# hanseongbugi/ORB_SLAM3_Study_kr

Measured on AMD Instinct MI355X. Metric: local-BA windows/sec (50 KF, 10k pts, 10 LM iters) + ORB matches/sec; 1/2/4/8 GPU, higher is better.
Workload: dtype f64; 1 GPU; BASELINE.json configs[1]: synthetic stereo local BA, 50 optimisable + 10 fixed KF, 10k landmarks (~75k stereo edges), optimize(10) with the reference's stop rules; windows_per_gpu=512, global_windows=512, streams_per_gpu=2, parallelism=independent windows, w mod 1

## Files before the change

### orb_slam3_study_kr_amd/csrc/lba_device.hip

```cpp
#include "common.h"
#include <type_traits>
#include <cstdlib>
#include <cstdio>
#include <atomic>
#include <chrono>
#include <thread>
#include "lba_math.h"
#include "ldlt_block.h"
#include "big_solve.h"
#include "schur_plan.h"
#include "lba_pack.h"
#include "lba_pack_device.h"
#include "g2o_lm.h"
#include <algorithm>
#include <cfloat>
#include <cmath>
#include <cstring>
#include <vector>

namespace osh {

constexpr int kResidualSplit = 1;
constexpr int kSolveThreadsBatch = 256, kSolveThreadsLatency = 512;
constexpr int kPoseRec = 21;
// ... 299 lines not shown
      const int e = pbase + tid;
      double hl[9];
#pragma unroll
      for (int k = 0; k < 9; ++k) hl[k] = 0.0;
      if (e < e1) {
        double qt[7], cam[5], R[9], X[3], Xc[3], Q[6], g[3], rho0;
        fetch_pose(staged, sh_pose, poses, cams, le.ip[p], qt, cam, R);
#pragma unroll
        for (int k = 0; k < 3; ++k) X[k] = sh_X[(le.il[p] - ch.lm0) * 3 + k];
        const double rec[4] = {le.ra[p].x, le.ra[p].y, le.rb[p].x, le.rb[p].y};
        win_edge_core<KB8>(wd, bv, (size_t)wd.edge_off + e, rec, qt, cam, R, X, Xc, Q, g, rho0);
        chi_acc += rho0;
        dev::core_landmark_side<KB8>(Q, g, R, hl);
      }
#pragma unroll
      for (int k = 0; k < 9; ++k) sh_c[k * kChunkEdges + tid] = hl[k];
      __syncthreads();
      if (tid < nl) {
        const int lo = max(my_lo, pbase), hi = min(my_hi, pbase + kChunkEdges);
        for (int x = lo; x < hi; ++x) {
#pragma unroll
          for (int k = 0; k < 9; ++k) acc[k] += sh_c[k * kChunkEdges + x - pbase];
        }
      }
      __syncthreads();
    }
  }
  double dmax = 0.0;
  if (tid < nl) {
    const size_t gl = (size_t)wd.pt_off + ch.lm0 + tid;
#pragma unroll
    for (int k = 0; k < 6; ++k) bv.Hll[gl * 6 + k] = acc[k];
#pragma unroll
    for (int k = 0; k < 3; ++k) bv.bl[gl * 3 + k] = acc[6 + k];
    dmax = fmax(fabs(acc[0]), fmax(fabs(acc[3]), fabs(acc[5])));
    if (lambda_known) {
      double dl[9];
      dev::landmark_factor(acc, acc + 6, st.lambda, dl);
#pragma unroll
      for (int k = 0; k < 9; ++k) bv.DL[gl * 9 + k] = dl[k];
    }
  }
  const double chi = block_sum(chi_acc, sh4);
  dmax = block_max(dmax, sh4);
  if (tid == 0) { bv.chi_lin[blockIdx.x] = chi; bv.dmax_lin[blockIdx.x] = dmax; }
}

typedef double f64x4 __attribute__((ext_vector_type(4)));
constexpr int kSiLm = 8;
constexpr int kSiRows = 6 * kItemPoses;
constexpr int kSiImage = 32 * 49;

template <bool SYM, bool KB8>
__global__ __launch_bounds__(64, KB8 ? 1 : 2) void k_schur_fused(BatchView bv, int item_base, int mode) {
  __shared__ double shA[(SYM && !KB8) ? kSiImage : kSiRows * (3 * kSiLm + 1)];
  __shared__ double shB[SYM ? 1 : kSiRows * (3 * kSiLm + 1)];
  __shared__ double shPose[(SYM ? 1 : 2) * 8 * kPoseRec];
  __shared__ int shP[64 + 8];
  const int item_idx = item_base + blockIdx.x;
  const SItem it = bv.sitems[item_idx];
  const WinDesc wd = bv.win[it.win];
  const LmView st = lm_view(bv.lm, it.win);
  if (!st.active) return;
  const bool do_hpp = SYM && (mode == 0 ? st.need_lin != 0 : (st.lin_now != 0 && st.iter > 0));
  const bool do_schur = mode != 0;
  if (!do_hpp && !do_schur) return;
  const int lane = threadIdx.x;
  const int nx = it.shape & 0xff, ny = (it.shape >> 8) & 0xff;
  const int TX = (6 * nx + 15) >> 4, TY = (6 * ny + 15) >> 4;
  shP[lane] = bv.spair[(size_t)item_idx * 64 + lane];
  if (lane < 8) shP[64 + lane] = bv.scslot[(size_t)item_idx * 8 + lane];
  {
    const double* poses = bv.pose_state[st.sel] + (size_t)wd.pose_off * 7;
    const double* cams = bv.pose_cam + (size_t)wd.pose_off * 5;
    const int side = lane >> 3, s8 = lane & 7;
    if (side < (SYM ? 1 : 2)) {
      const int ip = side == 0 ? bv.sposex[(size_t)item_idx * 8 + s8] : bv.sposey[(size_t)item_idx * 8 + s8];
      double qt[7], cam[5], Rm[9];
#pragma unroll
      for (int k = 0; k < 7; ++k) qt[k] = ip >= 0 ? poses[(size_t)ip * 7 + k] : 0.0;
#pragma unroll
      for (int k = 0; k < 5; ++k) cam[k] = ip >= 0 ? cams[(size_t)ip * 5 + k] : 0.0;
      dev::quat_to_R(qt, Rm);
      double* dst = shPose + (side * 8 + s8) * kPoseRec;
#pragma unroll
      for (int k = 0; k < 7; ++k) dst[k] = qt[k];
#pragma unroll
      for (int k = 0; k < 5; ++k) dst[7 + k] = cam[k];
#pragma unroll
      for (int k = 0; k < 9; ++k) dst[12 + k] = Rm[k];
    }
  }
  const SRec* __restrict__ recs = bv.srecs + it.rec_off;
  const double* pts = bv.pt_state[st.sel] + (size_t)wd.pt_off * 3;
  const double* DL = bv.DL + (size_t)wd.pt_off * 9;
  const int mrow = lane & 15, mk = lane >> 4;
  using std::integral_constant;

  auto body = [&](auto lmc, auto psc) __attribute__((always_inline)) {
    constexpr int LM = decltype(lmc)::value, PS = decltype(psc)::value;
    constexpr int KS = 3 * LM + 1;
    constexpr int KST = (3 * LM) / 4;
    static_assert(LM * PS <= 64 && (3 * LM) % 4 == 0 && ((6 * PS + 15) / 16) * 16 * KS <= ((SYM && !KB8) ? kSiImage : kSiRows * (3 * kSiLm + 1)), "chunk mapping");
    const int l = lane / PS, s = lane - l * PS;
    const bool lane_on = LM * PS == 64 || l < LM;
    f64x4 acc[3][3];
#pragma unroll
    for (int a = 0; a < 3; ++a)
#pragma unroll
      for (int b = 0; b < 3; ++b) acc[a][b] = (f64x4){0.0, 0.0, 0.0, 0.0};
    double csum[6] = {0, 0, 0, 0, 0, 0};
    double H[21], hb[6];
#pragma unroll
    for (int k = 0; k < 21; ++k) H[k] = 0.0;
#pragma unroll
    for (int k = 0; k < 6; ++k) hb[k] = 0.0;
    if (PS < 8) {
      for (int idx = lane; idx < (((6 * PS + 15) / 16) * 16 - 6 * PS) * KS; idx += 64) shA[6 * PS * KS + idx] = 0.0;
    }

    struct Dat { double2 ex[2]; double2 ey[2]; double X[3]; double dl[9]; };
    const int last_rec = it.n_lm - 1;
    const size_t last_edge = (size_t)wd.edge_off + (size_t)max(wd.E - 1, 0);
    auto load_rec = [&](int c0, int4& ra, int4& rb) {
      const int4* src = reinterpret_cast<const int4*>(recs + min(c0 + l, last_rec));
      ra = src[0]; rb = src[1];
    };
    auto slot_of = [&](unsigned lo, unsigned hi) { return (((s < 4) ? lo : hi) >> (8 * (s & 3))) & 0xffu; };
    auto edge_of = [&](const int4& ra, unsigned o) { return min((size_t)wd.edge_off + (size_t)(ra.y + (o != kAbsent ? (int)o : 0)), last_edge); };
    auto load_dat = [&](const int4& ra, const int4& rb, Dat& d) {
      const double2* src = reinterpret_cast<const double2*>(bv.e_rec + edge_of(ra, slot_of((unsigned)ra.z, (unsigned)ra.w)) * 4);
      d.ex[0] = src[0]; d.ex[1] = src[1];
      if (!SYM) {
        const double2* sy = reinterpret_cast<const double2*>(bv.e_rec + edge_of(ra, slot_of((unsigned)rb.x, (unsigned)rb.y)) * 4);
        d.ey[0] = sy[0]; d.ey[1] = sy[1];
      }
#pragma unroll
      for (int k = 0; k < 3; ++k) d.X[k] = pts[(size_t)ra.x * 3 + k];
      if (do_schur) {
#pragma unroll
        for (int k = 0; k < 9; ++k) d.dl[k] = DL[(size_t)ra.x * 9 + k];
      }
    };
    auto side_rows = [&](int side, bool present, const int4& ra, unsigned o, const double2* er, const Dat& d, double* img) __attribute__((always_inline)) {
      const double* ps = shPose + (side * 8 + s) * kPoseRec;
      double qt[7], cam[5], Rm[9];
#pragma unroll
      for (int k = 0; k < 7; ++k) qt[k] = ps[k];
#pragma unroll
      for (int k = 0; k < 5; ++k) cam[k] = ps[7 + k];
#pragma unroll
      for (int k = 0; k < 9; ++k) Rm[k] = ps[12 + k];
      const double rec[4] = {er[0].x, er[0].y, er[1].x, er[1].y};
      double Xc[3], Q[6], g[3], rho0;
      win_edge_core<KB8>(wd, bv, edge_of(ra, o), rec, qt, cam, Rm, d.X, Xc, Q, g, rho0);
#pragma unroll
      for (int k = 0; k < 6; ++k) Q[k] = present ? Q[k] : 0.0;
#pragma unroll
      for (int k = 0; k < 3; ++k) g[k] = present ? g[k] : 0.0;
      if (SYM && do_hpp && side == 0) dev::core_pose_side<KB8>(Xc, Q, g, H, hb);
      if (do_schur) {
        double WF[18];
        dev::core_WF<KB8>(Xc, Q, Rm, d.dl, WF);
        double* row = img + (6 * s) * KS + 3 * l;
        if (lane_on) {
#pragma unroll
          for (int r = 0; r < 6; ++r) { row[r * KS + 0] = WF[r * 3]; row[r * KS + 1] = WF[r * 3 + 1]; row[r * KS + 2] = WF[r * 3 + 2]; }
        }
        if (SYM) {
#pragma unroll
          for (int r = 0; r < 6; ++r) csum[r] += WF[r * 3] * d.dl[6] + WF[r * 3 + 1] * d.dl[7] + WF[r * 3 + 2] * d.dl[8];
        }
      }
    };
    auto park = [&](int c0, const int4& ra, const int4& rb, const Dat& d) __attribute__((always_inline)) {
      const bool valid = lane_on && (c0 + l) < it.n_lm;
      const unsigned xo = valid ? slot_of((unsigned)ra.z, (unsigned)ra.w) : kAbsent;
      wave_sync();
      side_rows(0, xo != kAbsent, ra, xo, d.ex, d, shA);
      if (!SYM) {
        const unsigned yo = valid ? slot_of((unsigned)rb.x, (unsigned)rb.y) : kAbsent;
        side_rows(1, yo != kAbsent, ra, yo, d.ey, d, shB);
      }
    };
    auto multiply_t = [&](auto txc, auto tyc) {
      constexpr int TXc = decltype(txc)::value, TYc = decltype(tyc)::value;
      const double* imgB = SYM ? shA : shB;
#pragma unroll
      for (int ks = 0; ks < KST; ++ks) {
        double a[3], b[3];
#pragma unroll
        for (int t = 0; t < 3; ++t) {
          a[t] = (t < TXc) ? shA[(16 * t + mrow) * KS + 4 * ks + mk] : 0.0;
          b[t] = SYM ? a[t] : ((t < TYc) ? imgB[(16 * t + mrow) * KS + 4 * ks + mk] : 0.0);
        }
#pragma unroll
        for (int ti = 0; ti < 3; ++ti)
#pragma unroll
          for (int tj = SYM ? ti : 0; tj < 3; ++tj)
            if (ti < TXc && tj < TYc) acc[ti][tj] = __builtin_amdgcn_mfma_f64_16x16x4f64(a[ti], b[tj], acc[ti][tj], 0, 0, 0);
        if (ks & 1) __builtin_amdgcn_sched_barrier(0);
      }
    };
    auto multiply_cross = [&]() {
#pragma unroll
      for (int ks = 0; ks < KST; ++ks) {
        double a[3], b[3];
#pragma unroll
        for (int t = 0; t < 3; ++t) {
          a[t] = (t < TX) ? shA[(16 * t + mrow) * KS + 4 * ks + mk] : 0.0;
          b[t] = (t < TY) ? shB[(16 * t + mrow) * KS + 4 * ks + mk] : 0.0;
        }
#pragma unroll
        for (int ti = 0; ti < 3; ++ti)
#pragma unroll
          for (int tj = 0; tj < 3; ++tj)
            if (ti < TX && tj < TY) acc[ti][tj] = __builtin_amdgcn_mfma_f64_16x16x4f64(a[ti], b[tj], acc[ti][tj], 0, 0, 0);
      }
    };
    int4 rc0, rc1, rn0, rn1;
    Dat d;
    load_rec(0, rc0, rc1);
    load_rec(LM, rn0, rn1);
    load_dat(rc0, rc1, d);
    wave_sync();
    auto chunk_loop = [&](auto txc) {
      for (int c0 = 0; c0 < it.n_lm; c0 += LM) {
        park(c0, rc0, rc1, d);
        wave_sync();
        rc0 = rn0; rc1 = rn1;
        load_dat(rc0, rc1, d);
        load_rec(c0 + 2 * LM, rn0, rn1);
        if (do_schur) {
          if (SYM) multiply_t(txc, txc); else multiply_cross();
        }
      }
    };
    if (SYM && do_schur) {
      if (PS > 5 && TX == 3) chunk_loop(integral_constant<int, 3>{});
      else if (PS > 2 && TX == 2) chunk_loop(integral_constant<int, 2>{});
      else chunk_loop(integral_constant<int, 1>{});
    } else {
      chunk_loop(integral_constant<int, 0>{});
    }
    wave_sync();
    if (do_schur) {
#pragma unroll
      for (int ti = 0; ti < 3; ++ti)
#pragma unroll
        for (int tj = SYM ? ti : 0; tj < 3; ++tj) {
          if (ti < TX && tj < TY) {
            const int C = 16 * tj + (lane & 15);
            const int sb = C / 6, cc = C - 6 * sb;
#pragma unroll
            for (int reg = 0; reg < 4; ++reg) {
              const int R = 16 * ti + (lane >> 4) + 4 * reg;
              const int sa = R / 6, rr = R - 6 * sa;
              const int slot = shP[sa * 8 + sb];
              if (slot >= 0) bv.contrib[(size_t)slot * 36 + rr * 6 + cc] = acc[ti][tj][reg];
            }
          }
        }
      if (SYM) {
        if (lane_on) {
#pragma unroll
          for (int r = 0; r < 6; ++r) shA[l * (6 * PS) + 6 * s + r] = csum[r];
        }
        wave_sync();
        if (lane < 6 * PS) {
          double v = 0.0;
#pragma unroll
          for (int k = 0; k < LM; ++k) v += shA[k * (6 * PS) + lane];
          const int sa = lane / 6;
          const int slot = shP[64 + sa];
          if (slot >= 0) bv.ccontrib[(size_t)slot * 6 + (lane - 6 * sa)] = v;
        }
        wave_sync();
      }
    }
    if (SYM && do_hpp) {
#pragma unroll
      for (int half = 0; half < 2; ++half) {
        const int k0 = half * 14, nk = half ? 13 : 14;
        wave_sync();
#pragma unroll
        for (int k = 0; k < 14; ++k) {
          const int kk = k0 + k;
          if (k < nk) shA[k * 64 + lane] = (kk < 21) ? H[kk < 21 ? kk : 0] : hb[(kk - 21) < 0 ? 0 : ((kk - 21) > 5 ? 5 : (kk - 21))];
        }
        wave_sync();
        for (int o = lane; o < PS * nk; o += 64) {
          const int k = o / PS, sa = o - k * PS;
          const int slot = shP[64 + sa];
          if (slot >= 0) {
            double v = 0.0;
#pragma unroll
            for (int ll = 0; ll < LM; ++ll) v += shA[k * 64 + ll * PS + sa];
            bv.hcontrib[(size_t)slot * 27 + k0 + k] = v;
          }
        }
      }
    }
  };
  if constexpr (SYM && !KB8) {
    if (nx <= 4) body(integral_constant<int, 16>{}, integral_constant<int, 4>{});
    else if (nx == 5) body(integral_constant<int, 12>{}, integral_constant<int, 5>{});
    else body(integral_constant<int, kSiLm>{}, integral_constant<int, 8>{});
  } else {
    body(integral_constant<int, kSiLm>{}, integral_constant<int, 8>{});
  }
}

template <bool DEEP>
__global__ __launch_bounds__(256) void k_schur_reduce(BatchView bv) {
  const int t = threadIdx.x / 36, el = threadIdx.x - 36 * t;
  const int idx = blockIdx.x * 7 + t;
  if (t >= 7 || idx >= bv.n_rblk) return;
  const RBlk rb = bv.rblk[idx];
  const WinDesc wd = bv.win[rb.win];
  const LmView st = lm_view(bv.lm, rb.win);
  if (!st.active) return;
  const int i = rb.ij & 0xffff, j = (rb.ij >> 16) & 0xffff;
  if (j == 0xffff) {
    if (el >= 6) return;
    const size_t gp = (size_t)wd.fpose_off + i;
    double v = bv.bp[gp * 6 + el];
    const double* c = bv.ccontrib + (size_t)rb.start * 6 + el;
    int k = 0;
    if constexpr (DEEP) {
      for (; k + 24 <= rb.count; k += 24) {
        double t[24];
#pragma unroll
        for (int u = 0; u < 24; ++u) t[u] = c[(size_t)(k + u) * 6];
        __builtin_amdgcn_sched_barrier(0);
#pragma unroll
        for (int u = 0; u < 24; ++u) v -= t[u];
      }
    }
    for (; k + 8 <= rb.count; k += 8) {
      double t[8];
#pragma unroll
      for (int u = 0; u < 8; ++u) t[u] = c[(size_t)(k + u) * 6];
      __builtin_amdgcn_sched_barrier(0);
#pragma unroll
      for (int u = 0; u < 8; ++u) v -= t[u];
    }
    for (; k < rb.count; ++k) v -= c[(size_t)k * 6];
    bv.bs[gp * 6 + el] = v;
    return;
  }
  if (bv.pose_lo && i < bv.pose_lo[wd.fpose_off + j]) return;
  const int r = el / 6, cc = el - 6 * r;
  double v = 0.0;
  if (i == j) v = bv.Hpp[((size_t)wd.fpose_off + i) * 36 + el] + ((r == cc) ? st.lambda : 0.0);
  const double* c = bv.contrib + (size_t)rb.start * 36 + el;
  int k = 0;
  if constexpr (DEEP) {
    for (; k + 24 <= rb.count; k += 24) {
      double t[24];
#pragma unroll
      for (int u = 0; u < 24; ++u) t[u] = c[(size_t)(k + u) * 36];
      __builtin_amdgcn_sched_barrier(0);
#pragma unroll
      for (int u = 0; u < 24; ++u) v -= t[u];
    }
  }
  for (; k + 8 <= rb.count; k += 8) {
    double t[8];
#pragma unroll
    for (int u = 0; u < 8; ++u) t[u] = c[(size_t)(k + u) * 36];
    __builtin_amdgcn_sched_barrier(0);
#pragma unroll
    for (int u = 0; u < 8; ++u) v -= t[u];
  }
  for (; k < rb.count; ++k) v -= c[(size_t)k * 36];
  bv.S[wd.S_off + (size_t)(6 * i + r) * wd.n + 6 * j + cc] = v;
}

__global__ __launch_bounds__(64) void k_pose_reduce(BatchView bv, int mode) {
  const int gp = blockIdx.x * 2 + (threadIdx.x >> 5);
  const int k = threadIdx.x & 31;
  if (gp >= bv.n_fposes) return;
  const int w = bv.fpose_win[gp];
  const LmView st = lm_view(bv.lm, w);
  if (!st.active || !(mode == 0 ? st.need_lin != 0 : (st.lin_now != 0 && st.iter > 0))) return;
  const I2 rg = bv.pose_crange[gp];
  double a = 0.0;
  if (k < 27) {
    const double* src = bv.hcontrib + (size_t)rg.x * 27 + k;
    int c = 0;
    for (; c + 16 <= rg.y; c += 16) {
      double t[16];
#pragma unroll
      for (int u = 0; u < 16; ++u) t[u] = src[(size_t)(c + u) * 27];
      __builtin_amdgcn_sched_barrier(0);
#pragma unroll
      for (int u = 0; u < 16; ++u) a += t[u];
    }
    for (; c + 4 <= rg.y; c += 4) {
      const double v0 = src[(size_t)c * 27], v1 = src[(size_t)(c + 1) * 27], v2 = src[(size_t)(c + 2) * 27], v3 = src[(size_t)(c + 3) * 27];
      a += v0; a += v1; a += v2; a += v3;
    }
    for (; c < rg.y; ++c) a += src[(size_t)c * 27];
    if (k < 21) {
      int r = 0, rem = k;
      while (rem >= 6 - r) { rem -= 6 - r; ++r; }
      const int cc = r + rem;
      double* Ho = bv.Hpp + (size_t)gp * 36;
      Ho[r * 6 + cc] = a;
      Ho[cc * 6 + r] = a;
    } else {
      bv.bp[(size_t)gp * 6 + (k - 21)] = a;
    }
  }
  __shared__ double shd[64];
  shd[threadIdx.x] = fabs(a);
  wave_sync();
  if (k == 0) {
    const double* d = shd + (threadIdx.x & 32);
    bv.dmax_pose[gp] = fmax(fmax(fmax(d[0], d[6]), fmax(d[11], d[15])), fmax(d[18], d[20]));
  }
}

template <int NT>
__device__ void solve_tail(BatchView& bv, const WinDesc& wd, LmState& st, const double* xs, double* shw, bool ok) {
  const int tid = threadIdx.x, n = wd.n;
  double* xp = bv.xp + (size_t)wd.fpose_off * 6;
  for (int k = tid; k < n; k += NT) xp[k] = xs[k];
  __syncthreads();
  const int cur = st.sel, tr_sel = st.sel ^ 1;
  const double lambda = st.lambda;
  double sc = 0.0;
  for (int i = tid; i < wd.P; i += NT) {
    double u[6], qin[7], qout[7];
#pragma unroll
    for (int k = 0; k < 6; ++k) u[k] = xs[6 * i + k];
#pragma unroll
    for (int k = 0; k < 7; ++k) qin[k] = bv.pose_state[cur][((size_t)wd.pose_off + i) * 7 + k];
    dev::pose_oplus(u, qin, qout);
#pragma unroll
    for (int k = 0; k < 7; ++k) bv.pose_state[tr_sel][((size_t)wd.pose_off + i) * 7 + k] = qout[k];
    const double* bpi = bv.bp + ((size_t)wd.fpose_off + i) * 6;
#pragma unroll
    for (int k = 0; k < 6; ++k) sc += u[k] * (lambda * u[k] + bpi[k]);
  }
  sc = dev::wave_sum(sc);
  if ((tid & 63) == 0) shw[tid >> 6] = sc;
  __syncthreads();
  if (tid == 0) {
    double tot = 0.0;
    for (int k = 0; k < NT / 64; ++k) tot += shw[k];
    st.scale_pose = tot; st.solve_ok = ok ? 1 : 0;
  }
}

template <int NB, int NT>
__global__ __launch_bounds__(NT) void k_solve(BatchView bv, int W) {
  constexpr int kSolveThreads = NT;
  extern __shared__ __attribute__((aligned(16))) double sh[];
  const int w = blockIdx.x;
  const WinDesc& wd = bv.win[w];
  LmState& st = bv.lm[w];
  if (!st.active) return;
  const int n = wd.n;
  double* A = bv.S + wd.S_off;
  double* rhs = bv.bs + (size_t)wd.fpose_off * 6;
  double *xs, *shw;
  const bool ok = ldlt_solve_block<NB, kSolveThreads>(A, rhs, n, W, sh, xs, shw, bv.pose_lo ? bv.pose_lo + wd.fpose_off : nullptr);
  solve_tail<kSolveThreads>(bv, wd, st, xs, shw, ok);
}

__global__ __launch_bounds__(256) void k_big_finish(BatchView bv, int w, const int* fail) {
  __shared__ double shw[8];
  const WinDesc& wd = bv.win[w];
  LmState& st = bv.lm[w];
  if (!st.active) return;
  double* x = bv.bs + (size_t)wd.fpose_off * 6;
  const bool ok = *fail == 0;
  if (!ok) {
    for (int k = threadIdx.x; k < wd.n; k += 256) x[k] = 0.0;
    __syncthreads();
  }
  solve_tail<256>(bv, wd, st, x, shw, ok);
}

template <bool KB8, bool F32>
__global__ __launch_bounds__(kBlock) void k_backsub(BatchView bv) {
  extern __shared__ __attribute__((aligned(16))) double sh_bs[];
  double* sh_c = sh_bs;
  double* sh4 = sh_bs + 3 * kChunkEdges;
  double* sh_X = sh4 + 4;
  double* sh_x = sh_X + 3 * kBlock;
  const Chunk ch = bv.chunks[blockIdx.x];
  const WinDesc wd = bv.win[ch.win];
  const LmView st = lm_view(bv.lm, ch.win);
  if (!st.active) return;
  const int tid = threadIdx.x;
  const int n = wd.n;
  const double* poses = bv.pose_state[st.sel] + (size_t)wd.pose_off * 7;
  const double* cams = bv.pose_cam + (size_t)wd.pose_off * 5;
  const double* pts = bv.pt_state[st.sel] + (size_t)wd.pt_off * 3;
  const bool staged = wd.P <= kLdsPoses;
  const double* xp = bv.xp + (size_t)wd.fpose_off * 6;
  double* sh_pose = sh_x + (staged ? n : 0);
  const int* lmo = bv.lm_off + wd.lmoff_off;
  const int e0 = lmo[ch.lm0], e1 = lmo[ch.lm1];
  const int nl = ch.lm1 - ch.lm0;
  const double lambda = st.lambda;
  double acc[3] = {0, 0, 0};
  int my_lo = 0, my_hi = 0;
  double F[6], b3[3], Xcur[3];
#pragma unroll
  for (int k = 0; k < 6; ++k) F[k] = 0.0;
  b3[0] = b3[1] = b3[2] = 0.0; Xcur[0] = Xcur[1] = Xcur[2] = 0.0;
  if (tid < nl) {
    const size_t gl = (size_t)wd.pt_off + ch.lm0 + tid;
    my_lo = lmo[ch.lm0 + tid]; my_hi = lmo[ch.lm0 + tid + 1];
#pragma unroll
    for (int k = 0; k < 6; ++k) F[k] = bv.DL[gl * 9 + k];
#pragma unroll
    for (int k = 0; k < 3; ++k) { b3[k] = bv.bl[gl * 3 + k]; Xcur[k] = pts[(size_t)(ch.lm0 + tid) * 3 + k]; }
  }
  for (int base = e0; base < e1; base += kChunkMaxEdges) {
    LaneEdges le;
    load_lane_edges<F32>(bv, wd, base, e1, tid, le);
    if (base == e0) {
      stage_points(sh_X, pts, ch.lm0, nl, tid);
      if (staged) {
        for (int k = tid; k < n; k += kBlock) sh_x[k] = xp[k];
        stage_poses(sh_pose, poses, cams, wd.P, tid, kBlock);
      }
      __syncthreads();
    }
#pragma unroll
    for (int p = 0; p < kPasses; ++p) {
      const int pbase = base + p * kChunkEdges;
      if (pbase >= e1) break;
      const int e = pbase + tid;
      double c[3] = {0, 0, 0};
      if (e < e1 && le.ip[p] < wd.P) {
        const int ip = le.ip[p];
        double qt[7], R[9], cam[5], X[3], Xc[3], Q[6], g[3], rho0, x6[6];
        fetch_pose(staged, sh_pose, poses, cams, ip, qt, cam, R);
#pragma unroll
        for (int k = 0; k < 6; ++k) x6[k] = staged ? sh_x[6 * ip + k] : xp[6 * ip + k];
#pragma unroll
        for (int k = 0; k < 3; ++k) X[k] = sh_X[(le.il[p] - ch.lm0) * 3 + k];
        const double rec[4] = {le.ra[p].x, le.ra[p].y, le.rb[p].x, le.rb[p].y};
        win_edge_core<KB8>(wd, bv, (size_t)wd.edge_off + e, rec, qt, cam, R, X, Xc, Q, g, rho0);
        dev::core_backsub<KB8>(Xc, Q, R, x6, c);
      }
      sh_c[tid] = c[0]; sh_c[kChunkEdges + tid] = c[1]; sh_c[2 * kChunkEdges + tid] = c[2];
      __syncthreads();
      if (tid < nl) {
        const int lo = max(my_lo, pbase), hi = min(my_hi, pbase + kChunkEdges);
        for (int x = lo; x < hi; ++x) {
          acc[0] += sh_c[x - pbase]; acc[1] += sh_c[kChunkEdges + x - pbase]; acc[2] += sh_c[2 * kChunkEdges + x - pbase];
        }
      }
      __syncthreads();
    }
  }
  double sc = 0.0;
  if (tid < nl) {
    const size_t gl = (size_t)wd.pt_off + ch.lm0 + tid;
    const double b0 = b3[0], b1 = b3[1], b2 = b3[2];
    const double c0 = b0 + acc[0], c1 = b1 + acc[1], c2 = b2 + acc[2];
    double xl[3];
    if (st.solve_ok) {
      const double t0 = F[0] * c0, t1 = F[1] * c0 + F[3] * c1, t2 = F[2] * c0 + F[4] * c1 + F[5] * c2;
      xl[0] = F[0] * t0 + F[1] * t1 + F[2] * t2;
      xl[1] = F[3] * t1 + F[4] * t2;
      xl[2] = F[5] * t2;
    } else {
      xl[0] = xl[1] = xl[2] = 0.0;
    }
    double* Xt = bv.pt_state[st.sel ^ 1] + gl * 3;
    Xt[0] = Xcur[0] + xl[0]; Xt[1] = Xcur[1] + xl[1]; Xt[2] = Xcur[2] + xl[2];
    sc = xl[0] * (lambda * xl[0] + b0) + xl[1] * (lambda * xl[1] + b1) + xl[2] * (lambda * xl[2] + b2);
  }
  sc = block_sum(sc, sh4);
  if (tid == 0) bv.scale_part[blockIdx.x] = sc;
  __syncthreads();
  if (tid < nl) {
    const double* Xt = bv.pt_state[st.sel ^ 1] + ((size_t)wd.pt_off + ch.lm0 + tid) * 3;
    sh_X[tid * 3] = Xt[0]; sh_X[tid * 3 + 1] = Xt[1]; sh_X[tid * 3 + 2] = Xt[2];
  }
  const double* poses_t = bv.pose_state[st.sel ^ 1] + (size_t)wd.pose_off * 7;
  const bool staged_t = (wd.P + wd.F) <= kLdsPoses;
  double* sh_pose_t = sh_pose + (staged ? wd.P * kPoseRec : 0);
  if (staged_t) stage_poses(sh_pose_t, poses_t, cams, wd.P + wd.F, tid, kBlock);
  __syncthreads();
  double chi_acc = 0.0;
  for (int base = e0; base < e1; base += kChunkMaxEdges) {
    LaneEdges le;
    load_lane_edges<F32>(bv, wd, base, e1, tid, le);
#pragma unroll
    for (int p = 0; p < kPasses; ++p) {
      const int e = base + p * kChunkEdges + tid;
      if (e < e1) {
        double qt[7], cam[5], R[9], X[3];
        fetch_pose(staged_t, sh_pose_t, poses_t, cams, le.ip[p], qt, cam, R);
#pragma unroll
        for (int k = 0; k < 3; ++k) X[k] = sh_X[(le.il[p] - ch.lm0) * 3 + k];
        const double rec[4] = {le.ra[p].x, le.ra[p].y, le.rb[p].x, le.rb[p].y};
        double cl, cr;
// ... 857 lines not shown
```

Before: 13070 windows/s.

## Add specialized cross-pair Schur kernel path for narrow column tiles with MFMA pipelining

Adds a dedicated code path for non-symmetric Schur off-diagonal blocks when the row tile has more than five poses and the column tile has at most four. It builds WF images for row and column poses in shared memory, software-pipelines record and data loads ahead of the compute passes, and accumulates with f64 MFMA tiles sized to the narrow column count. The aim is to avoid wasted MFMA work and padding that the generic 8x8 body spends on small column tiles. In exchange it adds a large specialised code path with more register pressure and extra indexing complexity.

```diff
diff --git a/orb_slam3_study_kr_amd/csrc/lba_device.hip b/orb_slam3_study_kr_amd/csrc/lba_device.hip
--- a/orb_slam3_study_kr_amd/csrc/lba_device.hip
+++ b/orb_slam3_study_kr_amd/csrc/lba_device.hip
@@ -625,6 +625,135 @@
       }
     }
   };
+  auto cross_pairs = [&](auto tyc) __attribute__((always_inline)) {
+    constexpr int TYc = decltype(tyc)::value;
+    constexpr int KS = 3 * kSiLm + 1, KSB = 3 * 16 + 1, KST = (3 * kSiLm) / 4;
+    static_assert(16 * TYc <= 32 && kSiRows * KS <= sizeof(shA) / sizeof(double) && 24 * KSB <= sizeof(shB) / sizeof(double), "image sizes");
+    const int l = lane >> 3, s = lane & 7;
+    const int lc = lane >> 2, sc = lane & 3;
+    f64x4 acc[3][TYc];
+#pragma unroll
+    for (int a = 0; a < 3; ++a)
+#pragma unroll
+      for (int b = 0; b < TYc; ++b) acc[a][b] = (f64x4){0.0, 0.0, 0.0, 0.0};
+
+    struct SDat { double2 e[2]; double X[3]; double dl[9]; };
+    const int last_rec = it.n_lm - 1;
+    const size_t last_edge = (size_t)wd.edge_off + (size_t)max(wd.E - 1, 0);
+    auto edge_of = [&](const int4& ra, unsigned o) { return min((size_t)wd.edge_off + (size_t)(ra.y + (o != kAbsent ? (int)o : 0)), last_edge); };
+    auto row_slot = [&](const int4& ra) { return (unsigned)((((unsigned long long)(unsigned)ra.w << 32) | (unsigned)ra.z) >> (8 * s)) & 0xffu; };
+    auto col_slot = [&](const int4& rb) { return ((unsigned)rb.x >> (8 * sc)) & 0xffu; };
+    auto load_row_rec = [&](int c0, int4& ra) { ra = *reinterpret_cast<const int4*>(recs + min(c0 + l, last_rec)); };
+    auto load_col_rec = [&](int p0, int4& ra, int4& rb) {
+      const int4* src = reinterpret_cast<const int4*>(recs + min(p0 + lc, last_rec));
+      ra = src[0]; rb = src[1];
+    };
+    auto load_dat = [&](const int4& ra, unsigned o, SDat& d) {
+      const double2* src = reinterpret_cast<const double2*>(bv.e_rec + edge_of(ra, o) * 4);
+      d.e[0] = src[0]; d.e[1] = src[1];
+#pragma unroll
+      for (int k = 0; k < 3; ++k) d.X[k] = pts[(size_t)ra.x * 3 + k];
+#pragma unroll
+      for (int k = 0; k < 9; ++k) d.dl[k] = DL[(size_t)ra.x * 9 + k];
+    };
+    auto wf_rows = [&](const double* ps, bool present, size_t ge, const SDat& d, double* row, int ks) __attribute__((always_inline)) {
+      double qt[7], cam[5], Rm[9];
+#pragma unroll
+      for (int k = 0; k < 7; ++k) qt[k] = ps[k];
+#pragma unroll
+      for (int k = 0; k < 5; ++k) cam[k] = ps[7 + k];
+#pragma unroll
+      for (int k = 0; k < 9; ++k) Rm[k] = ps[12 + k];
+      const double rec[4] = {d.e[0].x, d.e[0].y, d.e[1].x, d.e[1].y};
+      double Xc[3], Q[6], g[3], rho0;
+      win_edge_core<KB8>(wd, bv, ge, rec, qt, cam, Rm, d.X, Xc, Q, g, rho0);
+#pragma unroll
+      for (int k = 0; k < 6; ++k) Q[k] = present ? Q[k] : 0.0;
+      double WF[18];
+      dev::core_WF<KB8>(Xc, Q, Rm, d.dl, WF);
+#pragma unroll
+      for (int r = 0; r < 6; ++r) { row[r * ks + 0] = WF[r * 3]; row[r * ks + 1] = WF[r * 3 + 1]; row[r * ks + 2] = WF[r * 3 + 2]; }
+    };
+    auto row_pass = [&](int c0, const int4& ra, const SDat& d) __attribute__((always_inline)) {
+      const unsigned o = (c0 + l) < it.n_lm ? row_slot(ra) : kAbsent;
+      wf_rows(shPose + s * kPoseRec, o != kAbsent, edge_of(ra, o), d, shA + (6 * s) * KS + 3 * l, KS);
+    };
+    auto col_pass = [&](int p0, const int4& ra, const int4& rb, const SDat& d) __attribute__((always_inline)) {
+      const unsigned o = (p0 + lc) < it.n_lm ? col_slot(rb) : kAbsent;
+      wf_rows(shPose + (8 + sc) * kPoseRec, o != kAbsent, edge_of(ra, o), d, shB + (6 * sc) * KSB + 3 * lc, KSB);
+    };
+    auto multiply = [&](int cb) __attribute__((always_inline)) {
+#pragma unroll
+      for (int ks = 0; ks < KST; ++ks) {
+        double a[3], b[TYc];
+#pragma unroll
+        for (int t = 0; t < 3; ++t) a[t] = shA[(16 * t + mrow) * KS + 4 * ks + mk];
+#pragma unroll
+        for (int t = 0; t < TYc; ++t) b[t] = shB[min(16 * t + mrow, 23) * KSB + cb + 4 * ks + mk];
+#pragma unroll
+        for (int ti = 0; ti < 3; ++ti)
+#pragma unroll
+          for (int tj = 0; tj < TYc; ++tj) acc[ti][tj] = __builtin_amdgcn_mfma_f64_16x16x4f64(a[ti], b[tj], acc[ti][tj], 0, 0, 0);
+        if (ks & 1) __builtin_amdgcn_sched_barrier(0);
+      }
+    };
+    int4 rc, rn, cc0, cc1, cn0, cn1;
+    SDat rd, cd;
+    load_row_rec(0, rc);
+    load_col_rec(0, cc0, cc1);
+    load_row_rec(kSiLm, rn);
+    load_col_rec(2 * kSiLm, cn0, cn1);
+    load_dat(rc, row_slot(rc), rd);
+    load_dat(cc0, col_slot(cc1), cd);
+    wave_sync();
+    int p0 = 0;
+    for (; p0 + kSiLm < it.n_lm; p0 += 2 * kSiLm) {
+      wave_sync();
+      col_pass(p0, cc0, cc1, cd);
+      row_pass(p0, rc, rd);
+      wave_sync();
+      rc = rn;
+      load_dat(rc, row_slot(rc), rd);
+      load_row_rec(p0 + 2 * kSiLm, rn);
+      multiply(0);
+      wave_sync();
+      row_pass(p0 + kSiLm, rc, rd);
+      wave_sync();
+      rc = rn; cc0 = cn0; cc1 = cn1;
+      load_dat(rc, row_slot(rc), rd);
+      load_dat(cc0, col_slot(cc1), cd);
+      load_row_rec(p0 + 3 * kSiLm, rn);
+      load_col_rec(p0 + 4 * kSiLm, cn0, cn1);
+      multiply(3 * kSiLm);
+    }
+    if (p0 < it.n_lm) {
+      wave_sync();
+      col_pass(p0, cc0, cc1, cd);
+      row_pass(p0, rc, rd);
+      wave_sync();
+      multiply(0);
+    }
+#pragma unroll
+    for (int ti = 0; ti < 3; ++ti)
+#pragma unroll
+      for (int tj = 0; tj < TYc; ++tj) {
+        const int C = 16 * tj + (lane & 15);
+        const int sb = C / 6, cc = C - 6 * sb;
+#pragma unroll
+        for (int reg = 0; reg < 4; ++reg) {
+          const int R = 16 * ti + (lane >> 4) + 4 * reg;
+          const int sa = R / 6, rr = R - 6 * sa;
+          const int slot = shP[sa * 8 + sb];
+          if (slot >= 0) bv.contrib[(size_t)slot * 36 + rr * 6 + cc] = acc[ti][tj][reg];
+        }
+      }
+  };
+  if constexpr (!SYM && !KB8) {
+    if (nx > 5 && ny <= 4) {
+      if (ny <= 2) cross_pairs(integral_constant<int, 1>{}); else cross_pairs(integral_constant<int, 2>{});
+      return;
+    }
+  }
   if constexpr (SYM && !KB8) {
     if (nx <= 4) body(integral_constant<int, 16>{}, integral_constant<int, 4>{});
     else if (nx == 5) body(integral_constant<int, 12>{}, integral_constant<int, 5>{});
```

Result: faster. 13380 windows/s (median of 6 runs) (+2.4%).
